# halixness/distributed-3d-diffusion-pytorch

Measured on AMD Instinct MI355X. Metric: train imgs/sec (whole node), SRN cars 64x64 bs128, higher is better.
Workload: dtype bf16; 1 GPU; model=XUNet ch128 ch_mult(1,2,2,4) 136.7M params (3DiM, reference xunet.py), global_batch=128, seq_len=4096, image_size=64, per_gpu_batch=128, micro_batch=128, hip_graph=False, parallelism=dp1, dist_backend=none, tuned_gemms=True, backend=hip

## Files before the change

distributed_3d_diffusion_pytorch_amd/ops/csrc/attention.hip:

```cpp
#include "common.h"

typedef __attribute__((ext_vector_type(4))) short s16x4;
typedef __attribute__((ext_vector_type(8))) short s16x8;
typedef __attribute__((address_space(3))) s16x4 lds_s16x4;

namespace {

constexpr float LOG2E = 1.4426950408889634f;

__device__ __forceinline__ s16x4 ds_tr(const bf16* p) {
  return __builtin_amdgcn_ds_read_tr16_b64_v4i16((lds_s16x4*)(p));
}
__device__ __forceinline__ bf16x8 tr8(const bf16* base, int stride, int r1, int r2, int col) {
  s16x4 lo = ds_tr(base + r1 * stride + col);
  s16x4 hi = ds_tr(base + r2 * stride + col);
  s16x8 v = {lo[0], lo[1], lo[2], lo[3], hi[0], hi[1], hi[2], hi[3]};
  return __builtin_bit_cast(bf16x8, v);
}
__device__ __forceinline__ bf16x8 pack8(f32x4 a, f32x4 b) {
  bf16x8 r;
  r[0] = (bf16)a[0]; r[1] = (bf16)a[1]; r[2] = (bf16)a[2]; r[3] = (bf16)a[3];
  r[4] = (bf16)b[0]; r[5] = (bf16)b[1]; r[6] = (bf16)b[2]; r[7] = (bf16)b[3];
  return r;
}
template <int D>
__device__ __forceinline__ int swz(int row, int chunk) {
  return row * D + ((chunk ^ (row & 7)) << 3);
}

template <int D, bool KALL = false>
__global__ void __launch_bounds__(KALL ? 1024 : 256) attn_fwd_k(const bf16* __restrict__ qkv, bf16* __restrict__ out,
                                                               float* __restrict__ lse, int L, int C, int heads,
                                                               int cross, float scale) {
  constexpr int VS = D + 16;
  constexpr int KC = D / 32;
  constexpr int DT = D / 16;
  constexpr int KR = KALL ? 256 : 64, NT = KALL ? 1024 : 256;
  __shared__ __attribute__((aligned(16))) bf16 Ks[KR * D];
  __shared__ __attribute__((aligned(16))) bf16 Vs[KR * VS];
  const int tid = threadIdx.x, lane = tid & 63, w = tid >> 6;
  const int qblk = blockIdx.x, h = blockIdx.y, n = blockIdx.z;
  const int nkv = cross ? (n ^ 1) : n;
  const int g = lane >> 4, fr = lane & 15;
  const long C3 = 3L * C;
  const int q = qblk * (NT / 4) + w * 16 + fr;
  const bool qok = q < L;
  const bf16* qrow = qkv + ((long)n * L + (qok ? q : 0)) * C3 + h * D;
  bf16x8 qf[KC];
#pragma unroll
  for (int kc = 0; kc < KC; ++kc)
    qf[kc] = qok ? *reinterpret_cast<const bf16x8*>(qrow + 32 * kc + 8 * g) : bf16x8{};

  f32x4 o[DT];
#pragma unroll
  for (int t = 0; t < DT; ++t) o[t] = f32x4{0.f, 0.f, 0.f, 0.f};
  float m = -INFINITY, l = 0.f;
  const float sl2 = scale * LOG2E;
  const int qq = (lane & 15) >> 2, pc = lane & 3;

  constexpr int CH = D / 8;
  constexpr int NKV = KR * CH / NT;
  bf16x8 kr[NKV], vr[NKV];
  auto fetch = [&](int kb) {
#pragma unroll
    for (int i = 0; i < NKV; ++i) {
      int idx = tid + i * NT;
      int r = idx / CH, c = idx % CH;
      const bool kok = kb + r < L;
      const bf16* src = qkv + ((long)nkv * L + (kok ? kb + r : 0)) * C3 + h * D + c * 8;
      kr[i] = kok ? *reinterpret_cast<const bf16x8*>(src + C) : bf16x8{};
      vr[i] = kok ? *reinterpret_cast<const bf16x8*>(src + 2 * C) : bf16x8{};
    }
  };
  auto stage = [&]() {
#pragma unroll
    for (int i = 0; i < NKV; ++i) {
      int idx = tid + i * NT;
      int r = idx / CH, c = idx % CH;
      *reinterpret_cast<bf16x8*>(Ks + swz<D>(r, c)) = kr[i];
      *reinterpret_cast<bf16x8*>(Vs + r * VS + c * 8) = vr[i];
    }
  };
  fetch(0);
  if constexpr (KALL) {
    stage();
    __syncthreads();
    if (w * 16 >= L) return;
  }
  for (int kb = 0; kb < L; kb += 64) {
    if constexpr (!KALL) {
      stage();
      if (kb + 64 < L) fetch(kb + 64);
      __syncthreads();
    }
    const bf16* Kb = Ks + (KALL ? kb * D : 0);
    const bf16* Vb = Vs + (KALL ? kb * VS : 0);
    f32x4 s[4];
#pragma unroll
    for (int kt = 0; kt < 4; ++kt) {
      s[kt] = f32x4{0.f, 0.f, 0.f, 0.f};
#pragma unroll
      for (int kc = 0; kc < KC; ++kc) {
        bf16x8 a = *reinterpret_cast<const bf16x8*>(Kb + swz<D>(16 * kt + fr, 4 * kc + g));
        s[kt] = __builtin_amdgcn_mfma_f32_16x16x32_bf16(a, qf[kc], s[kt], 0, 0, 0);
      }
    }
    float mb = -INFINITY;
#pragma unroll
    for (int kt = 0; kt < 4; ++kt)
#pragma unroll
      for (int i = 0; i < 4; ++i) {
        s[kt][i] = kb + 16 * kt + 4 * g + i < L ? s[kt][i] * sl2 : -INFINITY;
        mb = fmaxf(mb, s[kt][i]);
      }
    mb = fmaxf(mb, __shfl_xor(mb, 16, 64));
    mb = fmaxf(mb, __shfl_xor(mb, 32, 64));
    float mn = fmaxf(m, mb);
    float alpha = exp2f(m - mn);
    float ls = 0.f;
#pragma unroll
    for (int kt = 0; kt < 4; ++kt)
#pragma unroll
      for (int i = 0; i < 4; ++i) {
        s[kt][i] = exp2f(s[kt][i] - mn);
        ls += s[kt][i];
      }
    ls += __shfl_xor(ls, 16, 64);
    ls += __shfl_xor(ls, 32, 64);
    l = l * alpha + ls;
    m = mn;
#pragma unroll
    for (int t = 0; t < DT; ++t) o[t] *= alpha;
#pragma unroll
    for (int kc2 = 0; kc2 < 2; ++kc2) {
      bf16x8 pb = pack8(s[2 * kc2], s[2 * kc2 + 1]);
      int r1 = 32 * kc2 + 4 * g + qq, r2 = 32 * kc2 + 16 + 4 * g + qq;
#pragma unroll
      for (int t = 0; t < DT; ++t) {
        bf16x8 va = tr8(Vb, VS, r1, r2, 16 * t + 4 * pc);
        o[t] = __builtin_amdgcn_mfma_f32_16x16x32_bf16(va, pb, o[t], 0, 0, 0);
      }
    }
    if constexpr (!KALL) __syncthreads();
  }
  if (!qok) return;
  const float inv = 1.f / l;
  bf16* orow = out + ((long)n * L + q) * C + h * D;
#pragma unroll
  for (int t = 0; t < DT; ++t) {
    bf16x4 v4;
#pragma unroll
    for (int i = 0; i < 4; ++i) v4[i] = (bf16)(o[t][i] * inv);
    *reinterpret_cast<bf16x4*>(orow + 16 * t + 4 * g) = v4;
  }
  if (g == 0) lse[((long)n * heads + h) * L + q] = (m + log2f(l)) / LOG2E;
}

template <int D, int KW = 64>
__global__ void __launch_bounds__(KW == 256 ? 512 : 256) attn_bwd_k(const bf16* __restrict__ qkv, const bf16* __restrict__ dout,
                                                     const float* __restrict__ lse, const bf16* __restrict__ out,
                                                     float* __restrict__ dq_acc, bf16* __restrict__ dqkv, int L, int C,
                                                     int heads, int cross, float scale) {
  constexpr int KC = D / 32, DT = D / 16;
  constexpr int NWV = KW == 256 ? 8 : 4, NT = 64 * NWV, KG = KW / (16 * NWV);
  constexpr int TS = D + 16;
  constexpr int SS = KW + 8;
  __shared__ __attribute__((aligned(16))) bf16 Qs[32 * TS];
  __shared__ __attribute__((aligned(16))) bf16 dOs[32 * TS];
  __shared__ __attribute__((aligned(16))) bf16 Kt[KW * TS];
  __shared__ __attribute__((aligned(16))) bf16 dSs[32 * SS];
  __shared__ float lse_s[32], D_s[32];
  const int tid = threadIdx.x, lane = tid & 63, w = tid >> 6;
  const int kblk = blockIdx.x, h = blockIdx.y, n = blockIdx.z;
  const int nkv = cross ? (n ^ 1) : n;
  const int g = lane >> 4, fr = lane & 15, qq = (lane & 15) >> 2, pc = lane & 3;
  const long C3 = 3L * C;
  const int k0 = kblk * KW;
  const float sl2 = scale * LOG2E;
  constexpr int CH = D / 8;

#pragma unroll
  for (int i = 0; i < KW * CH / NT; ++i) {
    int idx = tid + i * NT;
    int r = idx / CH, c = idx % CH;
    *reinterpret_cast<bf16x8*>(Kt + r * TS + c * 8) =
        k0 + r < L ? *reinterpret_cast<const bf16x8*>(qkv + ((long)nkv * L + k0 + r) * C3 + C + h * D + c * 8)
                   : bf16x8{};
  }
  bool kok[KG];
  bf16x8 kf[KG][KC], vf[KG][KC];
  f32x4 dk[KG][DT], dv[KG][DT];
#pragma unroll
  for (int kg = 0; kg < KG; ++kg) {
    const int key = k0 + 16 * (w + NWV * kg) + fr;
    kok[kg] = key < L;
    const bf16* krow = qkv + ((long)nkv * L + (kok[kg] ? key : 0)) * C3 + h * D;
#pragma unroll
    for (int kc = 0; kc < KC; ++kc) {
      kf[kg][kc] = kok[kg] ? *reinterpret_cast<const bf16x8*>(krow + C + 32 * kc + 8 * g) : bf16x8{};
      vf[kg][kc] = kok[kg] ? *reinterpret_cast<const bf16x8*>(krow + 2 * C + 32 * kc + 8 * g) : bf16x8{};
    }
#pragma unroll
    for (int t = 0; t < DT; ++t) {
      dk[kg][t] = f32x4{0.f, 0.f, 0.f, 0.f};
      dv[kg][t] = f32x4{0.f, 0.f, 0.f, 0.f};
    }
  }
  const float* lse_nh = lse + ((long)n * heads + h) * L;
  const bool direct_dq = L <= KW;

  constexpr int NQ = (32 * CH + NT - 1) / NT;
  constexpr int PER = D / 8;
  bf16x8 qr[NQ], dr[NQ], orr[PER / 8], drr[PER / 8];
  float lse_r = 0.f;
  bool lse_ok = false;
  auto fetch = [&](int qb) {
#pragma unroll
    for (int i = 0; i < NQ; ++i) {
      int idx = tid + i * NT;
      int r = idx / CH, c = idx % CH;
      const bool ok = idx < 32 * CH && qb + r < L;
      long row = (long)n * L + (ok ? qb + r : 0);
      qr[i] = ok ? *reinterpret_cast<const bf16x8*>(qkv + row * C3 + h * D + c * 8) : bf16x8{};
      dr[i] = ok ? *reinterpret_cast<const bf16x8*>(dout + row * C + h * D + c * 8) : bf16x8{};
    }
    {
      const int r = tid >> 3, part = tid & 7;
      const bool ok = r < 32 && qb + r < L;
      const long row = (long)n * L + (ok ? qb + r : 0);
#pragma unroll
      for (int k = 0; k < PER / 8; ++k) {
        orr[k] = ok ? *reinterpret_cast<const bf16x8*>(out + row * C + h * D + part * PER + 8 * k) : bf16x8{};
        drr[k] = ok ? *reinterpret_cast<const bf16x8*>(dout + row * C + h * D + part * PER + 8 * k) : bf16x8{};
      }
    }
    const int li = qb + (tid & 31);
    lse_ok = tid < 32 && li < L;
    lse_r = lse_nh[li < L ? li : 0];
  };
  fetch(0);

  for (int q0 = 0; q0 < L; q0 += 32) {
    __syncthreads();
#pragma unroll
    for (int i = 0; i < NQ; ++i) {
      int idx = tid + i * NT;
      if (idx < 32 * CH) {
        int r = idx / CH, c = idx % CH;
        *reinterpret_cast<bf16x8*>(Qs + r * TS + c * 8) = qr[i];
        *reinterpret_cast<bf16x8*>(dOs + r * TS + c * 8) = dr[i];
      }
    }
    if (tid < 32) lse_s[tid] = lse_ok ? lse_r * LOG2E : INFINITY;
    {
      const int r = tid >> 3, part = tid & 7;
      float acc = 0.f;
#pragma unroll
      for (int k = 0; k < PER / 8; ++k)
#pragma unroll
        for (int j = 0; j < 8; ++j) acc += (float)orr[k][j] * (float)drr[k][j];
      acc += __shfl_xor(acc, 1, 64);
      acc += __shfl_xor(acc, 2, 64);
      acc += __shfl_xor(acc, 4, 64);
      if (part == 0 && r < 32) D_s[r] = acc;
    }
    if (q0 + 32 < L) fetch(q0 + 32);
    __syncthreads();
#pragma unroll
    for (int kg = 0; kg < KG; ++kg) {
      f32x4 p[2], ds[2];
#pragma unroll
      for (int qt = 0; qt < 2; ++qt) {
        f32x4 s = {0.f, 0.f, 0.f, 0.f}, dp = {0.f, 0.f, 0.f, 0.f};
#pragma unroll
        for (int kc = 0; kc < KC; ++kc) {
          bf16x8 a = *reinterpret_cast<const bf16x8*>(Qs + (16 * qt + fr) * TS + 32 * kc + 8 * g);
          s = __builtin_amdgcn_mfma_f32_16x16x32_bf16(a, kf[kg][kc], s, 0, 0, 0);
          bf16x8 b = *reinterpret_cast<const bf16x8*>(dOs + (16 * qt + fr) * TS + 32 * kc + 8 * g);
          dp = __builtin_amdgcn_mfma_f32_16x16x32_bf16(b, vf[kg][kc], dp, 0, 0, 0);
        }
#pragma unroll
        for (int i = 0; i < 4; ++i) {
          int qi = 16 * qt + 4 * g + i;
          float pv = kok[kg] ? exp2f(s[i] * sl2 - lse_s[qi]) : 0.f;
          p[qt][i] = pv;
          ds[qt][i] = pv * (dp[i] - D_s[qi]);
        }
      }
      bf16x8 pa = pack8(p[0], p[1]);
      bf16x8 dsa = pack8(ds[0], ds[1]);
      int r1 = 4 * g + qq, r2 = 16 + 4 * g + qq;
#pragma unroll
      for (int t = 0; t < DT; ++t) {
        bf16x8 bo = tr8(dOs, TS, r1, r2, 16 * t + 4 * pc);
        dv[kg][t] = __builtin_amdgcn_mfma_f32_16x16x32_bf16(pa, bo, dv[kg][t], 0, 0, 0);
        bf16x8 bq = tr8(Qs, TS, r1, r2, 16 * t + 4 * pc);
        dk[kg][t] = __builtin_amdgcn_mfma_f32_16x16x32_bf16(dsa, bq, dk[kg][t], 0, 0, 0);
      }
      {
        const int kl = 16 * (w + NWV * kg) + fr, u = kl & 31;
        const int col = (kl & ~31) + (u < 16 ? 8 * (u >> 2) + (u & 3) : 8 * ((u - 16) >> 2) + 4 + (u & 3));
#pragma unroll
        for (int qt = 0; qt < 2; ++qt)
#pragma unroll
          for (int i = 0; i < 4; ++i) dSs[(16 * qt + 4 * g + i) * SS + col] = (bf16)ds[qt][i];
      }
    }
    __syncthreads();
    for (int tt = w; tt < 2 * DT; tt += NWV) {
      int qt = tt / DT, t = tt % DT;
      f32x4 acc = {0.f, 0.f, 0.f, 0.f};
#pragma unroll
      for (int kc = 0; kc < KW / 32; ++kc) {
        bf16x8 a = *reinterpret_cast<const bf16x8*>(dSs + (16 * qt + fr) * SS + 32 * kc + 8 * g);
        bf16x8 b = tr8(Kt, TS, 32 * kc + 4 * g + qq, 32 * kc + 16 + 4 * g + qq, 16 * t + 4 * pc);
        acc = __builtin_amdgcn_mfma_f32_16x16x32_bf16(a, b, acc, 0, 0, 0);
      }
      if (direct_dq) {
#pragma unroll
        for (int i = 0; i < 4; ++i) {
          if (q0 + 16 * qt + 4 * g + i >= L) continue;
          long row = (long)n * L + q0 + 16 * qt + 4 * g + i;
          dqkv[row * C3 + h * D + 16 * t + fr] = (bf16)(acc[i] * scale);
        }
      } else {
        float* slab = dq_acc + (long)kblk * gridDim.z * L * C;
#pragma unroll
        for (int i = 0; i < 4; ++i) {
          if (q0 + 16 * qt + 4 * g + i >= L) continue;
          long row = (long)n * L + q0 + 16 * qt + 4 * g + i;
          slab[row * C + h * D + 16 * t + fr] = acc[i] * scale;
        }
      }
    }
  }
#pragma unroll
  for (int kg = 0; kg < KG; ++kg)
#pragma unroll
    for (int t = 0; t < DT; ++t)
#pragma unroll
      for (int i = 0; i < 4; ++i) {
        const int kk = k0 + 16 * (w + NWV * kg) + 4 * g + i;
        if (kk >= L) continue;
        long row = (long)nkv * L + kk;
        dqkv[row * C3 + C + h * D + 16 * t + fr] = (bf16)(dk[kg][t][i] * scale);
        dqkv[row * C3 + 2 * C + h * D + 16 * t + fr] = (bf16)dv[kg][t][i];
      }
}

__global__ void dq_convert_k(const float* __restrict__ dq, bf16* __restrict__ dqkv, long rows, int C, int kb) {
  const long total = rows * C / 8, slab = rows * C;
  for (long i = blockIdx.x * (long)blockDim.x + threadIdx.x; i < total; i += (long)gridDim.x * blockDim.x) {
    long r = (i * 8) / C;
    int c = (int)((i * 8) % C);
    f32x8 s = ld8f(dq + i * 8);
    for (int k = 1; k < kb; ++k) s += ld8f(dq + k * slab + i * 8);
    st8(dqkv + r * 3L * C + c, s);
  }
}

}

static int g_attn_fwd_all_min = 512;
D3D_API void d3d_attn_fwd_cfg(int min_pairs) { g_attn_fwd_all_min = min_pairs; }
D3D_API int d3d_attn_fwd(const void* qkv, void* out, float* lse, int N, int L, int C, int heads, int cross,
                         float scale, hipStream_t st) {
  int D = C / heads;
  if (L < 1) return (int)hipErrorInvalidValue;
  if (D == 64 && L > 64 && L <= 256 && N * heads >= g_attn_fwd_all_min) {
    hipLaunchKernelGGL((attn_fwd_k<64, true>), dim3(1, heads, N), dim3(1024), 0, st, (const bf16*)qkv, (bf16*)out, lse,
                       L, C, heads, cross, scale);
    return (int)hipGetLastError();
  }
  dim3 grid((L + 63) / 64, heads, N);
  if (D == 64)
    hipLaunchKernelGGL(attn_fwd_k<64>, grid, dim3(256), 0, st, (const bf16*)qkv, (bf16*)out, lse, L, C, heads, cross,
                       scale);
  else if (D == 128)
    hipLaunchKernelGGL(attn_fwd_k<128>, grid, dim3(256), 0, st, (const bf16*)qkv, (bf16*)out, lse, L, C, heads,
                       cross, scale);
  else
    return (int)hipErrorInvalidValue;
  return (int)hipGetLastError();
}

static long g_attn_wide_min = 0;
D3D_API void d3d_attn_bwd_cfg(int wide_min_pairs) { g_attn_wide_min = wide_min_pairs; }
static bool attn_wide(int N, int L, int C, int heads) {
  return heads > 0 && C / heads == 64 && L > 64 && L <= 256 && (long)N * heads >= g_attn_wide_min;
}
D3D_API int d3d_attn_bwd_slabs(int N, int L, int C, int heads) {
  return (L <= 64 || attn_wide(N, L, C, heads)) ? 0 : (L + 63) / 64;
}

D3D_API int d3d_attn_bwd(const void* qkv, const void* out, const void* dout, const float* lse, float* dq_acc,
                         void* dqkv, int N, int L, int C, int heads, int cross, float scale, hipStream_t st) {
  int D = C / heads;
  const int slabs = d3d_attn_bwd_slabs(N, L, C, heads);
  if (L < 1 || (slabs > 0 && dq_acc == nullptr)) return (int)hipErrorInvalidValue;
  if (attn_wide(N, L, C, heads)) {
    hipLaunchKernelGGL((attn_bwd_k<64, 256>), dim3(1, heads, N), dim3(512), 0, st, (const bf16*)qkv,
                       (const bf16*)dout, lse, (const bf16*)out, dq_acc, (bf16*)dqkv, L, C, heads, cross, scale);
    return (int)hipGetLastError();
  }
  const int kblocks = (L + 63) / 64;
  dim3 grid(kblocks, heads, N);
  if (D == 64)
    hipLaunchKernelGGL(attn_bwd_k<64>, grid, dim3(256), 0, st, (const bf16*)qkv, (const bf16*)dout, lse,
                       (const bf16*)out, dq_acc, (bf16*)dqkv, L, C, heads, cross, scale);
  else if (D == 128)
    hipLaunchKernelGGL(attn_bwd_k<128>, grid, dim3(256), 0, st, (const bf16*)qkv, (const bf16*)dout, lse,
                       (const bf16*)out, dq_acc, (bf16*)dqkv, L, C, heads, cross, scale);
  else
    return (int)hipErrorInvalidValue;
  if (L <= 64) return (int)hipGetLastError();
  long rows = (long)N * L;
  long g = (rows * C / 8 + 255) / 256;
  if (g > 4096) g = 4096;
  hipLaunchKernelGGL(dq_convert_k, dim3((int)g), dim3(256), 0, st, dq_acc, (bf16*)dqkv, rows, C, kblocks);
  return (int)hipGetLastError();
}
```

Before: 1134 examples/s.

## Restructure attention backward with 64-row query tiles, double buffering and transposed dS

Rewrites the flash-attention backward kernel to process 64 query rows per iteration instead of 32. For the 256-key variant it double-buffers the Q/dO tiles so the next tile is staged while the current one is computed. The softmax LSE and the row-dot D are folded into the MFMA accumulator initial values, the dS tile is stored transposed so dQ can read it with transpose loads, and dK/dV/dQ writes use permlane16 swaps to produce 16-byte vector stores. The kernel also gains a launch-bounds occupancy hint of 2 blocks. The aim is fewer barriers per key block and better latency hiding, at the cost of more LDS and register pressure.

```diff
diff --git a/distributed_3d_diffusion_pytorch_amd/ops/csrc/attention.hip b/distributed_3d_diffusion_pytorch_amd/ops/csrc/attention.hip
--- a/distributed_3d_diffusion_pytorch_amd/ops/csrc/attention.hip
+++ b/distributed_3d_diffusion_pytorch_amd/ops/csrc/attention.hip
@@ -156,20 +156,40 @@
   if (g == 0) lse[((long)n * heads + h) * L + q] = (m + log2f(l)) / LOG2E;
 }
 
+typedef unsigned u32x2 __attribute__((ext_vector_type(2)));
+typedef unsigned u32x4 __attribute__((ext_vector_type(4)));
+
+__device__ __forceinline__ void store_pair16(bf16* p, bool ok, f32x4 x, f32x4 y, float sc, int g) {
+  bf16x4 ox, oy;
+#pragma unroll
+  for (int i = 0; i < 4; ++i) {
+    ox[i] = (bf16)(x[i] * sc);
+    oy[i] = (bf16)(y[i] * sc);
+  }
+  const u32x2 ux = __builtin_bit_cast(u32x2, ox), uy = __builtin_bit_cast(u32x2, oy);
+  const auto s0 = __builtin_amdgcn_permlane16_swap(ux[0], uy[0], false, false);
+  const auto s1 = __builtin_amdgcn_permlane16_swap(ux[1], uy[1], false, false);
+  const u32x4 v = {s0[0], s1[0], s0[1], s1[1]};
+  if (ok) *reinterpret_cast<u32x4*>(p + 16 * (g & 1) + 8 * (g >> 1)) = v;
+}
+
 template <int D, int KW = 64>
-__global__ void __launch_bounds__(KW == 256 ? 512 : 256) attn_bwd_k(const bf16* __restrict__ qkv, const bf16* __restrict__ dout,
+__global__ void __launch_bounds__(KW == 256 ? 512 : 256, 2) attn_bwd_k(const bf16* __restrict__ qkv, const bf16* __restrict__ dout,
                                                      const float* __restrict__ lse, const bf16* __restrict__ out,
                                                      float* __restrict__ dq_acc, bf16* __restrict__ dqkv, int L, int C,
                                                      int heads, int cross, float scale) {
   constexpr int KC = D / 32, DT = D / 16;
   constexpr int NWV = KW == 256 ? 8 : 4, NT = 64 * NWV, KG = KW / (16 * NWV);
+  constexpr int QT = 64;
+  constexpr int NB = KW == 256 ? 2 : 1;
   constexpr int TS = D + 16;
-  constexpr int SS = KW + 8;
-  __shared__ __attribute__((aligned(16))) bf16 Qs[32 * TS];
-  __shared__ __attribute__((aligned(16))) bf16 dOs[32 * TS];
+  constexpr int SQ = QT + 8;
+  constexpr int TPW = DT / (NWV / 4);
+  __shared__ __attribute__((aligned(16))) bf16 Qs[NB * QT * TS];
+  __shared__ __attribute__((aligned(16))) bf16 dOs[NB * QT * TS];
   __shared__ __attribute__((aligned(16))) bf16 Kt[KW * TS];
-  __shared__ __attribute__((aligned(16))) bf16 dSs[32 * SS];
-  __shared__ float lse_s[32], D_s[32];
+  __shared__ __attribute__((aligned(16))) bf16 dSt[NB * KW * SQ];
+  __shared__ __attribute__((aligned(16))) float ls_s[NB * QT], D_s[NB * QT];
   const int tid = threadIdx.x, lane = tid & 63, w = tid >> 6;
   const int kblk = blockIdx.x, h = blockIdx.y, n = blockIdx.z;
   const int nkv = cross ? (n ^ 1) : n;
@@ -208,144 +228,162 @@
   }
   const float* lse_nh = lse + ((long)n * heads + h) * L;
   const bool direct_dq = L <= KW;
-
-  constexpr int NQ = (32 * CH + NT - 1) / NT;
-  constexpr int PER = D / 8;
-  bf16x8 qr[NQ], dr[NQ], orr[PER / 8], drr[PER / 8];
+  const int nkc = ((L - k0 < KW ? L - k0 : KW) + 31) / 32;
+
+  constexpr int NQ = QT * CH / NT;
+  bf16x8 qr[NQ], dr[NQ], orr[NQ];
   float lse_r = 0.f;
   bool lse_ok = false;
   auto fetch = [&](int qb) {
 #pragma unroll
     for (int i = 0; i < NQ; ++i) {
-      int idx = tid + i * NT;
-      int r = idx / CH, c = idx % CH;
-      const bool ok = idx < 32 * CH && qb + r < L;
-      long row = (long)n * L + (ok ? qb + r : 0);
+      const int idx = tid + i * NT;
+      const int r = idx / CH, c = idx % CH;
+      const bool ok = qb + r < L;
+      const long row = (long)n * L + (ok ? qb + r : 0);
       qr[i] = ok ? *reinterpret_cast<const bf16x8*>(qkv + row * C3 + h * D + c * 8) : bf16x8{};
       dr[i] = ok ? *reinterpret_cast<const bf16x8*>(dout + row * C + h * D + c * 8) : bf16x8{};
-    }
-    {
-      const int r = tid >> 3, part = tid & 7;
-      const bool ok = r < 32 && qb + r < L;
-      const long row = (long)n * L + (ok ? qb + r : 0);
-#pragma unroll
-      for (int k = 0; k < PER / 8; ++k) {
-        orr[k] = ok ? *reinterpret_cast<const bf16x8*>(out + row * C + h * D + part * PER + 8 * k) : bf16x8{};
-        drr[k] = ok ? *reinterpret_cast<const bf16x8*>(dout + row * C + h * D + part * PER + 8 * k) : bf16x8{};
-      }
-    }
-    const int li = qb + (tid & 31);
-    lse_ok = tid < 32 && li < L;
+      orr[i] = ok ? *reinterpret_cast<const bf16x8*>(out + row * C + h * D + c * 8) : bf16x8{};
+    }
+    const int li = qb + (tid & (QT - 1));
+    lse_ok = tid < QT && li < L;
     lse_r = lse_nh[li < L ? li : 0];
   };
+  auto stage = [&](int buf) {
+#pragma unroll
+    for (int i = 0; i < NQ; ++i) {
+      const int idx = tid + i * NT;
+      const int r = idx / CH, c = idx % CH;
+      *reinterpret_cast<bf16x8*>(Qs + (buf * QT + r) * TS + c * 8) = qr[i];
+      *reinterpret_cast<bf16x8*>(dOs + (buf * QT + r) * TS + c * 8) = dr[i];
+      float acc = 0.f;
+#pragma unroll
+      for (int j = 0; j < 8; ++j) acc += (float)orr[i][j] * (float)dr[i][j];
+#pragma unroll
+      for (int m = 1; m < CH; m <<= 1) acc += __shfl_xor(acc, m, 64);
+      if (c == 0) D_s[buf * QT + r] = -acc;
+    }
+    if (tid < QT) ls_s[buf * QT + tid] = lse_ok ? -lse_r / scale : -INFINITY;
+  };
   fetch(0);
-
-  for (int q0 = 0; q0 < L; q0 += 32) {
+  stage(0);
+  if constexpr (NB == 2) {
+    if (QT < L) fetch(QT);
+  }
+  __syncthreads();
+
+  for (int q0 = 0, cur = 0; q0 < L; q0 += QT, cur ^= NB - 1) {
+    const bool more = q0 + QT < L;
+    const bf16* Qb = Qs + cur * QT * TS;
+    const bf16* dOb = dOs + cur * QT * TS;
+    bf16* dSb = dSt + cur * KW * SQ;
+#pragma unroll
+    for (int c = 0; c < 2; ++c) {
+      bf16x8 pa[KG], dsa[KG];
+#pragma unroll
+      for (int hq = 0; hq < 2; ++hq) {
+        const int qt = 2 * c + hq;
+        bf16x8 aq[KC], ad[KC];
+#pragma unroll
+        for (int kc = 0; kc < KC; ++kc) {
+          aq[kc] = *reinterpret_cast<const bf16x8*>(Qb + (16 * qt + fr) * TS + 32 * kc + 8 * g);
+          ad[kc] = *reinterpret_cast<const bf16x8*>(dOb + (16 * qt + fr) * TS + 32 * kc + 8 * g);
+        }
+        const f32x4 l4 = *reinterpret_cast<const f32x4*>(ls_s + cur * QT + 16 * qt + 4 * g);
+        const f32x4 d4 = *reinterpret_cast<const f32x4*>(D_s + cur * QT + 16 * qt + 4 * g);
+#pragma unroll
+        for (int kg = 0; kg < KG; ++kg) {
+          f32x4 s = l4, dp = d4;
+#pragma unroll
+          for (int kc = 0; kc < KC; ++kc) {
+            s = __builtin_amdgcn_mfma_f32_16x16x32_bf16(aq[kc], kf[kg][kc], s, 0, 0, 0);
+            dp = __builtin_amdgcn_mfma_f32_16x16x32_bf16(ad[kc], vf[kg][kc], dp, 0, 0, 0);
+          }
+          bf16x4 ds4;
+#pragma unroll
+          for (int i = 0; i < 4; ++i) {
+            const float pv = kok[kg] ? exp2f(s[i] * sl2) : 0.f;
+            const float dsv = pv * dp[i];
+            pa[kg][4 * hq + i] = (bf16)pv;
+            dsa[kg][4 * hq + i] = (bf16)dsv;
+            ds4[i] = (bf16)dsv;
+          }
+          *reinterpret_cast<bf16x4*>(dSb + (16 * (w + NWV * kg) + fr) * SQ + 16 * qt + 4 * g) = ds4;
+        }
+      }
+      const int r1 = 32 * c + 4 * g + qq, r2 = 32 * c + 16 + 4 * g + qq;
+#pragma unroll
+      for (int t = 0; t < DT; ++t) {
+        const bf16x8 bo = tr8(dOb, TS, r1, r2, 16 * t + 4 * pc);
+        const bf16x8 bq = tr8(Qb, TS, r1, r2, 16 * t + 4 * pc);
+#pragma unroll
+        for (int kg = 0; kg < KG; ++kg) {
+          dv[kg][t] = __builtin_amdgcn_mfma_f32_16x16x32_bf16(bo, pa[kg], dv[kg][t], 0, 0, 0);
+          dk[kg][t] = __builtin_amdgcn_mfma_f32_16x16x32_bf16(bq, dsa[kg], dk[kg][t], 0, 0, 0);
+        }
+      }
+    }
+    if constexpr (NB == 2) {
+      if (more) {
+        stage(cur ^ 1);
+        if (q0 + 2 * QT < L) fetch(q0 + 2 * QT);
+      }
+    }
     __syncthreads();
-#pragma unroll
-    for (int i = 0; i < NQ; ++i) {
-      int idx = tid + i * NT;
-      if (idx < 32 * CH) {
-        int r = idx / CH, c = idx % CH;
-        *reinterpret_cast<bf16x8*>(Qs + r * TS + c * 8) = qr[i];
-        *reinterpret_cast<bf16x8*>(dOs + r * TS + c * 8) = dr[i];
-      }
-    }
-    if (tid < 32) lse_s[tid] = lse_ok ? lse_r * LOG2E : INFINITY;
+    if constexpr (NB == 1) {
+      if (more) fetch(q0 + QT);
+    }
     {
-      const int r = tid >> 3, part = tid & 7;
-      float acc = 0.f;
-#pragma unroll
-      for (int k = 0; k < PER / 8; ++k)
-#pragma unroll
-        for (int j = 0; j < 8; ++j) acc += (float)orr[k][j] * (float)drr[k][j];
-      acc += __shfl_xor(acc, 1, 64);
-      acc += __shfl_xor(acc, 2, 64);
-      acc += __shfl_xor(acc, 4, 64);
-      if (part == 0 && r < 32) D_s[r] = acc;
-    }
-    if (q0 + 32 < L) fetch(q0 + 32);
-    __syncthreads();
-#pragma unroll
-    for (int kg = 0; kg < KG; ++kg) {
-      f32x4 p[2], ds[2];
-#pragma unroll
-      for (int qt = 0; qt < 2; ++qt) {
-        f32x4 s = {0.f, 0.f, 0.f, 0.f}, dp = {0.f, 0.f, 0.f, 0.f};
-#pragma unroll
-        for (int kc = 0; kc < KC; ++kc) {
-          bf16x8 a = *reinterpret_cast<const bf16x8*>(Qs + (16 * qt + fr) * TS + 32 * kc + 8 * g);
-          s = __builtin_amdgcn_mfma_f32_16x16x32_bf16(a, kf[kg][kc], s, 0, 0, 0);
-          bf16x8 b = *reinterpret_cast<const bf16x8*>(dOs + (16 * qt + fr) * TS + 32 * kc + 8 * g);
-          dp = __builtin_amdgcn_mfma_f32_16x16x32_bf16(b, vf[kg][kc], dp, 0, 0, 0);
+      constexpr int TPB = TPW > 4 ? 4 : TPW;
+      const int qt = w & 3;
+      const int q = q0 + 16 * qt + fr;
+      const bool ok = q < L;
+      const long row = (long)n * L + (ok ? q : 0);
+#pragma unroll
+      for (int u0 = 0; u0 < TPW; u0 += TPB) {
+        const int t0 = (w >> 2) * TPW + u0;
+        f32x4 acc[TPB];
+#pragma unroll
+        for (int u = 0; u < TPB; ++u) acc[u] = f32x4{0.f, 0.f, 0.f, 0.f};
+        for (int kc = 0; kc < nkc; ++kc) {
+          const int r1 = 32 * kc + 4 * g + qq, r2 = r1 + 16;
+          const bf16x8 b = tr8(dSb, SQ, r1, r2, 16 * qt + 4 * pc);
+#pragma unroll
+          for (int u = 0; u < TPB; ++u) {
+            const bf16x8 a = tr8(Kt, TS, r1, r2, 16 * (t0 + u) + 4 * pc);
+            acc[u] = __builtin_amdgcn_mfma_f32_16x16x32_bf16(a, b, acc[u], 0, 0, 0);
+          }
         }
-#pragma unroll
-        for (int i = 0; i < 4; ++i) {
-          int qi = 16 * qt + 4 * g + i;
-          float pv = kok[kg] ? exp2f(s[i] * sl2 - lse_s[qi]) : 0.f;
-          p[qt][i] = pv;
-          ds[qt][i] = pv * (dp[i] - D_s[qi]);
+        if (direct_dq) {
+#pragma unroll
+          for (int u = 0; u < TPB; u += 2)
+            store_pair16(dqkv + row * C3 + h * D + 16 * (t0 + u), ok, acc[u], acc[u + 1], scale, g);
+        } else {
+          float* slab = dq_acc + (long)kblk * gridDim.z * L * C;
+#pragma unroll
+          for (int u = 0; u < TPB; ++u)
+            if (ok) *reinterpret_cast<f32x4*>(slab + row * C + h * D + 16 * (t0 + u) + 4 * g) = acc[u] * scale;
         }
       }
-      bf16x8 pa = pack8(p[0], p[1]);
-      bf16x8 dsa = pack8(ds[0], ds[1]);
-      int r1 = 4 * g + qq, r2 = 16 + 4 * g + qq;
-#pragma unroll
-      for (int t = 0; t < DT; ++t) {
-        bf16x8 bo = tr8(dOs, TS, r1, r2, 16 * t + 4 * pc);
-        dv[kg][t] = __builtin_amdgcn_mfma_f32_16x16x32_bf16(pa, bo, dv[kg][t], 0, 0, 0);
-        bf16x8 bq = tr8(Qs, TS, r1, r2, 16 * t + 4 * pc);
-        dk[kg][t] = __builtin_amdgcn_mfma_f32_16x16x32_bf16(dsa, bq, dk[kg][t], 0, 0, 0);
-      }
-      {
-        const int kl = 16 * (w + NWV * kg) + fr, u = kl & 31;
-        const int col = (kl & ~31) + (u < 16 ? 8 * (u >> 2) + (u & 3) : 8 * ((u - 16) >> 2) + 4 + (u & 3));
-#pragma unroll
-        for (int qt = 0; qt < 2; ++qt)
-#pragma unroll
-          for (int i = 0; i < 4; ++i) dSs[(16 * qt + 4 * g + i) * SS + col] = (bf16)ds[qt][i];
-      }
-    }
-    __syncthreads();
-    for (int tt = w; tt < 2 * DT; tt += NWV) {
-      int qt = tt / DT, t = tt % DT;
-      f32x4 acc = {0.f, 0.f, 0.f, 0.f};
-#pragma unroll
-      for (int kc = 0; kc < KW / 32; ++kc) {
-        bf16x8 a = *reinterpret_cast<const bf16x8*>(dSs + (16 * qt + fr) * SS + 32 * kc + 8 * g);
-        bf16x8 b = tr8(Kt, TS, 32 * kc + 4 * g + qq, 32 * kc + 16 + 4 * g + qq, 16 * t + 4 * pc);
-        acc = __builtin_amdgcn_mfma_f32_16x16x32_bf16(a, b, acc, 0, 0, 0);
-      }
-      if (direct_dq) {
-#pragma unroll
-        for (int i = 0; i < 4; ++i) {
-          if (q0 + 16 * qt + 4 * g + i >= L) continue;
-          long row = (long)n * L + q0 + 16 * qt + 4 * g + i;
-          dqkv[row * C3 + h * D + 16 * t + fr] = (bf16)(acc[i] * scale);
-        }
-      } else {
-        float* slab = dq_acc + (long)kblk * gridDim.z * L * C;
-#pragma unroll
-        for (int i = 0; i < 4; ++i) {
-          if (q0 + 16 * qt + 4 * g + i >= L) continue;
-          long row = (long)n * L + q0 + 16 * qt + 4 * g + i;
-          slab[row * C + h * D + 16 * t + fr] = acc[i] * scale;
-        }
-      }
-    }
-  }
-#pragma unroll
-  for (int kg = 0; kg < KG; ++kg)
-#pragma unroll
-    for (int t = 0; t < DT; ++t)
-#pragma unroll
-      for (int i = 0; i < 4; ++i) {
-        const int kk = k0 + 16 * (w + NWV * kg) + 4 * g + i;
-        if (kk >= L) continue;
-        long row = (long)nkv * L + kk;
-        dqkv[row * C3 + C + h * D + 16 * t + fr] = (bf16)(dk[kg][t][i] * scale);
-        dqkv[row * C3 + 2 * C + h * D + 16 * t + fr] = (bf16)dv[kg][t][i];
-      }
+    }
+    if constexpr (NB == 1) {
+      if (more) {
+        stage(0);
+        __syncthreads();
+      }
+    }
+  }
+#pragma unroll
+  for (int kg = 0; kg < KG; ++kg) {
+    const int kk = k0 + 16 * (w + NWV * kg) + fr;
+    const bool ok = kk < L;
+    bf16* krow = dqkv + ((long)nkv * L + (ok ? kk : 0)) * C3 + C + h * D;
+#pragma unroll
+    for (int t = 0; t < DT; t += 2) {
+      store_pair16(krow + 16 * t, ok, dk[kg][t], dk[kg][t + 1], scale, g);
+      store_pair16(krow + C + 16 * t, ok, dv[kg][t], dv[kg][t + 1], 1.f, g);
+    }
+  }
 }
 
 __global__ void dq_convert_k(const float* __restrict__ dq, bf16* __restrict__ dqkv, long rows, int C, int kb) {
```

After: 1123 examples/s. About the same (-0.9%).
